# CSTR-Edinburgh/magphase

Hardware: AMD Instinct MI355X
Metric: frames/sec analysis+synthesis @48kHz FFT=4096 (higher is better)
Workload: dtype f32

## Files before the change

### include/magphase_hip.h

```cpp
#ifndef MAGPHASE_HIP_H
#define MAGPHASE_HIP_H

#include <stddef.h>
#include <stdint.h>

#ifdef __cplusplus
extern "C" {
#endif

#define MPX_ABI_VERSION 2

#define MPX_OK 0
#define MPX_ERR_ARG (-1)
#define MPX_ERR_HIP (-2)
#define MPX_ERR_HOST (-3)

int mpx_version(void);
const char* mpx_last_error(void);

size_t mpx_tables_bytes(int fft_len);
int mpx_tables_init(void* stream, int fft_len, void* tables);

int mpx_analysis_frames(void* stream, int fft_len, const void* tables, const float* sig,
                        const int64_t* frame_pos, const int32_t* frame_left, const int32_t* frame_right,
                        int64_t n_frames, float* out_mag, float* out_real, float* out_imag, int64_t ld);

size_t mpx_tables_f64_bytes(int fft_len);
int mpx_tables_f64_init(void* stream, int fft_len, void* tables);
int mpx_analysis_frames_f64(void* stream, int fft_len, const void* tables_f64, const float* sig,
                            const int64_t* frame_pos, const int32_t* frame_left, const int32_t* frame_right,
                            int64_t n_frames, float* out_mag, float* out_real, float* out_imag, int64_t ld,
                            const float* rows_in_use);

int mpx_analysis_frames_f64w(void* stream, int fft_len, const void* tables_f64, const float* sig,
                             const int64_t* frame_pos, const int32_t* frame_left, const int32_t* frame_right,
                             int64_t n_frames, float* out_mag, float* out_real, float* out_imag, int64_t ld,
                             const float* rows_in_use, const double* win_tab, int32_t win_cap);

int mpx_analysis_compressed_fused(void* stream, int fft_len, const void* tables_f64, const float* sig,
                                  const int64_t* frame_pos, const int32_t* frame_left, const int32_t* frame_right,
                                  int64_t n_frames, const double* win_tab, int32_t win_cap, const float* wpack,
                                  const float* whalf, int32_t mag_dim, int32_t phase_dim, const float* voiced,
                                  int32_t mag_fbank, float* out_mag, float* out_real, float* out_imag);
int mpx_analysis_compressed_fused_cr(void* stream, int fft_len, const void* tables_f64, const float* sig,
                                     const int64_t* frame_pos, const int32_t* frame_left, const int32_t* frame_right,
                                     int64_t n_frames, const double* win_tab, int32_t win_cap, const float* wpack,
                                     const float* whalf, int32_t mag_dim, int32_t phase_dim, const float* rows_in_use,
                                     const int32_t* row0, const int32_t* row1, const float* row_t, int64_t n_const,
// ... 359 lines not shown
```

### magphase_amd/_lib.py

```python
import ctypes
import threading
import os

_HERE = os.path.dirname(os.path.abspath(__file__))
LIB_PATH = os.path.join(_HERE, "libmagphase_hip.so")

vp, i32, i64, sz, f64 = ctypes.c_void_p, ctypes.c_int32, ctypes.c_int64, ctypes.c_size_t, ctypes.c_double
u32 = ctypes.c_uint32

PROTOTYPES = {
    "mpx_version": (i32, []),
    "mpx_last_error": (ctypes.c_char_p, []),
    "mpx_tables_bytes": (sz, [i32]),
    "mpx_tables_init": (i32, [vp, i32, vp]),
    "mpx_feat_ld": (i64, [i32]),
    "mpx_analysis_frames": (i32, [vp, i32] + [vp] * 5 + [i64, vp, vp, vp, i64]),
    "mpx_tables_f64_bytes": (sz, [i32]),
    "mpx_tables_f64_init": (i32, [vp, i32, vp]),
    "mpx_analysis_frames_f64": (i32, [vp, i32] + [vp] * 5 + [i64, vp, vp, vp, i64, vp]),
    "mpx_analysis_frames_f64w": (i32, [vp, i32] + [vp] * 5 + [i64, vp, vp, vp, i64, vp, vp, i32]),
    "mpx_analysis_compressed_fused": (i32, [vp, i32] + [vp] * 5 + [i64, vp, i32, vp, vp, i32, i32, vp, i32, vp, vp,
                                       vp]),
    "mpx_analysis_compressed_fused_cr": (i32, [vp, i32] + [vp] * 5 + [i64, vp, i32, vp, vp, i32, i32] + [vp] * 4 +
                                          [i64] + [vp] * 4),
    "mpx_analysis_compressed_fused_cr_work_bytes": (i64, [i32, i64]),
    "mpx_analysis_compressed_fused_tiles": (i32, [i32, i32, ctypes.POINTER(i32), ctypes.POINTER(i32)]),
    "mpx_analysis_compressed_fused_waves": (i32, []),
    "mpx_analysis_compressed_fused_layout": (i32, []),
    "mpx_analysis_compressed_fused_blocks_per_cu": (i32, [i32, i32]),
    "mpx_synthesis_lossless_frames": (i32, [vp, i32] + [vp] * 4 + [i64, vp, i64]),
    "mpx_ola_gather": (i32, [vp, i32, vp, i32] + [vp] * 4 + [i64, vp]),
    "mpx_synth_ola_slots": (i32, []),
    "mpx_synth_ola_slot_weights": (i32, [vp, i32]),
    "mpx_ola_strip_floats": (i64, [i32]),
    "mpx_synthesis_lossless_ola": (i32, [vp, i32] + [vp] * 5 + [i32, vp, vp, i32, vp, vp, vp, i64]),
    "mpx_synthesis_lossless_ola_lerp": (i32, [vp, i32] + [vp] * 8 + [i32, vp, vp, i32, vp, vp, vp, i64]),
    "mpx_rows_lerp": (i32, [vp, i32, vp, vp, vp, i64, vp, vp, vp, i64, vp, vp, vp, i64]),
    "mpx_synthesis_lossless_backward": (i32, [vp, i32, vp, vp, i64, vp, vp, vp, i64, vp, vp, vp, i64] + [vp] * 6 + [i64]),
    "mpx_synthesis_compressed_backward": (i32, [vp, i32, vp, vp, i64, vp, vp, vp, i64, vp, vp, vp, i64] + [vp] * 12
# ... 57 lines not shown
    "mpx_mel_unwarp_backward": (i32, [vp, i32, vp, i64, vp, i64, vp, i32, i64, vp, vp, vp, i64, i32, vp, i32, i64, vp, vp]),
    "mpx_phase_grad_mask": (i32, [vp, i64, i32] + [vp] * 7),
    "mpx_min_phase": (i32, [vp, i32] + [vp] * 5 + [i64, vp, vp, vp, i64]),
    "mpx_true_envelope": (i32, [vp, i32, vp, vp, vp, i64, i64, i32, f64, i32, vp, i64, vp, vp, vp]),
    "mpx_frame_gain": (i32, [vp, i32] + [vp] * 5 + [i64, vp, i32]),
    "mpx_noise_gains": (i32, [vp] * 4 + [i32, i32, vp, vp]),
    "mpx_noise_power": (i32, [vp, i32] + [vp] * 5 + [i64, vp]),
    "mpx_noise_rms": (i32, [vp, i32, vp, vp, i32, vp, vp]),
    "mpx_post_filter": (i32, [vp, vp, i64, i32, vp, i32, i32, vp, vp]),
    "mpx_epoch_f0_track": (i32, [vp, vp, vp, i32, i32, vp, i64, vp, vp, vp, i64] + [i32] * 4 + [f64, vp, vp, vp]),
    "mpx_epoch_zff": (i32, [vp, vp, vp, i32, i64, vp, i32, vp, vp, vp, i32] + [vp] * 5),
    "mpx_pcm16": (i32, [vp, vp, i32, vp, i32, i64, f64, vp, vp]),
    "mpx_pcm16_to_f32": (i32, [vp, vp, i64, vp]),
    "mpx_hpf_block": (i32, []),
    "mpx_output_hpf": (i32, [vp] * 4 + [i32, i64] + [vp] * 7),
    "mpx_bw_probe": (i32, [vp, i32, vp, vp, i64]),
    "mpx_bw_probe_shapes": (i32, []),
    "mpx_rows_pack": (i32, [vp, vp, vp, i32, i32] + [vp, i32, i64, i64] * 3),
    "mpx_post_filter_merlin": (i32, [vp, vp, i64, i32] + [vp] * 4 + [i32, f64, vp, f64] + [vp] * 5),
}
SYMBOLS = tuple(PROTOTYPES)
RT_STORE_FLAGS = {"rows": 4, "lines": 0, "lines_nt": 8}
RT_INVERSE_FLAGS = {"direct": 0, "transform": 32}
del vp, i32, i64, sz, f64

_lib = None


class MagphaseHipError(RuntimeError):
    pass


_load_lock = threading.Lock()


def load():
    global _lib
    if _lib is not None:
        return _lib
    with _load_lock:
        return _load_locked()


def _load_locked():
    global _lib
    if _lib is not None:
# ... 20 lines not shown
```

### magphase_amd/autograd.py

```python
import torch
from torch.autograd.function import once_differentiable


class _LosslessSynthesis(torch.autograd.Function):

    @staticmethod
    def forward(ctx, plan, cat_fn, n_utts, *mats):
        feats = [tuple(mats[3 * u:3 * u + 3]) for u in range(n_utts)]
        cat = cat_fn(feats)
        pcm = plan.run(cat[0], cat[1], cat[2])
        ctx.plan = plan
        ctx.rows = [int(f[0].shape[0]) for f in feats]
        ctx.like = [(m.dtype, tuple(m.shape)) if torch.is_tensor(m) else None for m in mats]
        ctx.save_for_backward(*cat)
        return pcm

    @staticmethod
    @once_differentiable
    def backward(ctx, grad_out):
        mag, real, imag = ctx.saved_tensors
        n_head = 3
        need_in = ctx.needs_input_grad[n_head:]
        need = tuple(any(need_in[k::3]) for k in range(3))
        if grad_out.dtype != torch.float32 or not grad_out.is_contiguous():
# ... 1 lines not shown
        with torch.cuda.device(grad_out.device):
            g = ctx.plan.run_backward(grad_out, mag, real, imag, need=need)
        out, a = [], 0
        for u, n in enumerate(ctx.rows):
            for k in range(3):
                like = ctx.like[3 * u + k]
                if like is None or not need_in[3 * u + k]:
                    out.append(None)
                else:
                    out.append(g[k][a:a + n].to(like[0]).reshape(like[1]))
            a += n
        return (None,) * n_head + tuple(out)


def synthesize(plan, cat_fn, feats):
    mats = [x for f in feats for x in f[:3]]
    return _LosslessSynthesis.apply(plan, cat_fn, len(feats), *mats)


class _LosslessAnalysis(torch.autograd.Function):

    @staticmethod
    def forward(ctx, plan, *sigs):
        mag, real, imag = plan.run()
        ctx.plan = plan
        ctx.like = [(s.dtype, tuple(s.shape)) if torch.is_tensor(s) else None for s in sigs]
        ctx.set_materialize_grads(False)
        ctx.save_for_backward(mag, real, imag)
        return mag, real, imag

    @staticmethod
    @once_differentiable
    def backward(ctx, *grads):
        mag, real, imag = ctx.saved_tensors
        need_in = ctx.needs_input_grad[1:]
        grads = tuple(g if g is None or (g.dtype == torch.float32 and g.is_contiguous())
                      else g.to(torch.float32).contiguous() for g in grads)
        with torch.cuda.device(mag.device):
            gsig = ctx.plan.run_backward(mag, real, imag, grads)
        out, a = [], 0
        for like, need, n in zip(ctx.like, need_in, ctx.plan.n_smpls):
            out.append(gsig[a:a + n].to(like[0]).reshape(like[1]) if like is not None and need else None)
            a += n
        return (None,) + tuple(out)


def analyze(plan, sigs):
# ... 112 lines not shown
```

### magphase_amd/csrc/magphase_hip.hip

```cpp
#include "mpx_common.hpp"

namespace mpx {

#ifdef MPX_ANA_NT
#define MPX_ST(dst, val) __builtin_nontemporal_store((val), &(dst))
#else
#define MPX_ST(dst, val) ((dst) = (val))
#endif

#ifndef MPX_ANA_QUEUE
#define MPX_ANA_QUEUE 0
#endif
template <int P>
__global__ __launch_bounds__(kAnaThreads) void k_analysis(const float* __restrict__ sig,
                                                          const long long* __restrict__ fpos,
                                                          const int* __restrict__ fleft,
                                                          const int* __restrict__ fright, long long nframes,
                                                          const float* __restrict__ tw_g, float* __restrict__ omag,
                                                          float* __restrict__ oreal, float* __restrict__ oimag,
                                                          long long ld) {
    constexpr int M = 64 * P, N = 2 * M, LB = ilog2(P), kTile = 64 * P;
    extern __shared__ __attribute__((aligned(16))) float smem[];
    float* tw = smem;
    const int lane_id = threadIdx.x & 63;
    const int wave = threadIdx.x >> 6;
    float* xbuf = smem + tw_floats<P>() + wave * (P * kXStride);
    const unsigned xbuf_byte = 4u * (unsigned)(tw_floats<P>() + rfl(wave) * (P * kXStride));
    for (int i = threadIdx.x; i < tw_floats<P>(); i += kAnaThreads) tw[i] = tw_g[i];
    unsigned* queue = reinterpret_cast<unsigned*>(smem + tw_floats<P>() + kAnaWaves * (P * kXStride));
    if (threadIdx.x == 0) *queue = 0u;
    __syncthreads();

    float wl_s0, wl_c0;
    sincospif(-2.0f * (float)kappa<P>(lane_id) / (float)N, &wl_s0, &wl_c0);

#if MPX_ANA_QUEUE
// ... 56 lines not shown
            }
            wave_sync();
        }

        wave_fft_front<P, -1>(re, im, tw, xbuf, lane);

#if MPX_ANA_QUEUE
        const long long fn = queue_pull(queue, fb);
#else
        const long long fn = f + fstep;
#endif
        FrameGeom gn = g;
        if (fn < fe) {
            gn = frame_geom(sig, fpos[fn], fleft[fn], fright[fn], N);
            asm volatile("s_waitcnt lgkmcnt(0)" ::: "memory");
            stage_samples_async(gn, 0, kTile, xbuf_byte, lane);
        }

        fft_inreg<P, -1>(re, im);

        float* row_m = omag + f * ld;
        float* row_r = oreal + f * ld;
        float* row_i = oimag + f * ld;
        float* mlo = row_m + kap;
        float* rlo = row_r + kap;
        float* ilo = row_i + kap;
        const int hoff = lane0 ? M - 64 : M - kap;
        float* mhi = row_m + hoff;
        float* rhi = row_r + hoff;
        float* ihi = row_i + hoff;
        float zpr[P / 2], zpi[P / 2];
#pragma unroll
        for (int q = 0; q < P / 2; ++q) {
            const int i = brev(q, LB);
            zpr[q] = __shfl(re[P - 1 - i], src_lane);
            zpi[q] = __shfl(im[P - 1 - i], src_lane);
        }
        float hm = 0.0f, hr = 0.0f, hi_ = 0.0f;
#pragma unroll
        for (int q = 0; q < P / 2; ++q) {
            const int i = brev(q, LB);
            const int i0 = brev((P - q) % P, LB);
            const float pr = lane0 ? re[i0] : zpr[q];
            const float pi = lane0 ? im[i0] : zpi[q];
            const float er = 0.5f * (re[i] + pr), ei = 0.5f * (im[i] - pi);
            const float orr = 0.5f * (im[i] + pi), oi = -0.5f * (re[i] - pr);
            const float cq = cos2p<P>(q), sq = -sin2p<P>(q);
            const float wr = wl_c * cq - wl_s * sq, wi = wl_c * sq + wl_s * cq;
            const float tr = wr * orr - wi * oi, ti = wr * oi + wi * orr;
            {
                const float xr = er + tr, xi = ei + ti;
                const float s2 = xr * xr + xi * xi;
                const float r = __builtin_amdgcn_rsqf(fmaxf(s2, 1.0e-37f));
#ifdef MPX_PROBE_NOSTORE
                asm volatile("" ::"v"(s2 * r), "v"(xr * r), "v"(xi * r));
#else
                MPX_ST(mlo[64 * q], s2 * r);
                MPX_ST(rlo[64 * q], xr * r);
                MPX_ST(ilo[64 * q], xi * r);
#endif
            }
            {
                const float xr = er - tr, xi = ti - ei;
                const float s2 = xr * xr + xi * xi;
                const float r = __builtin_amdgcn_rsqf(fmaxf(s2, 1.0e-37f));
                const float cm = s2 * r, cr = xr * r, ci = xi * r;
#ifdef MPX_PROBE_NOSTORE
                asm volatile("" ::"v"(cm), "v"(cr), "v"(ci));
#else
                if (q == 0) {
                    if (lane0) {
                        MPX_ST(row_m[M], cm);
                        MPX_ST(row_r[M], cr);
                        MPX_ST(row_i[M], ci);
                    }
                } else {
                    MPX_ST(mhi[-64 * (q - 1)], lane0 ? cm : hm);
                    MPX_ST(rhi[-64 * (q - 1)], lane0 ? cr : hr);
                    MPX_ST(ihi[-64 * (q - 1)], lane0 ? ci : hi_);
                }
#endif
                hm = cm;
                hr = cr;
                hi_ = ci;
            }
        }
        {
            const float xr = re[1], xi = -im[1];
            const float s2 = xr * xr + xi * xi;
            const float r = __builtin_amdgcn_rsqf(fmaxf(s2, 1.0e-37f));
#ifdef MPX_PROBE_NOSTORE
            asm volatile("" ::"v"(s2 * r), "v"(xr * r), "v"(xi * r), "v"(hm), "v"(hr), "v"(hi_));
#else
            MPX_ST(mhi[-64 * (P / 2 - 1)], lane0 ? s2 * r : hm);
            MPX_ST(rhi[-64 * (P / 2 - 1)], lane0 ? xr * r : hr);
            MPX_ST(ihi[-64 * (P / 2 - 1)], lane0 ? xi * r : hi_);
#endif
        }
        g = gn;
        if (fn >= fe) break;
#ifdef MPX_PROBE_NOSTORE
        staged_wait<0>();
#else
        staged_wait<3 * P + 3>();
#endif
        f = fn;
    }
}

template <int P>
__global__ __launch_bounds__(kThreads) void k_synth_lossless(const float* __restrict__ mag,
                                                             const float* __restrict__ real,
                                                             const float* __restrict__ imag, long long nframes,
                                                             const float* __restrict__ tw_g,
                                                             float* __restrict__ frames, long long ld) {
    constexpr int M = 64 * P, N = 2 * M, H = M + 1, LB = ilog2(P);
    extern __shared__ __attribute__((aligned(16))) float smem[];
    float* tw = smem;
    const int lane_id = threadIdx.x & 63;
    const int wave = threadIdx.x >> 6;
    float* xbuf = smem + tw_floats<P>() + wave * (P * kXStride);
    for (int i = threadIdx.x; i < tw_floats<P>(); i += kThreads) tw[i] = tw_g[i];
    __syncthreads();

    float wl_s0, wl_c0;
    sincospif(2.0f * (float)lane_id / (float)N, &wl_s0, &wl_c0);

// ... 557 lines not shown
        return fail(MPX_ERR_ARG, "mpx_analysis_frames: null pointer%s");
    const dim3 grid(grid_for(n_frames, kAnaWaves)), block(kAnaThreads);
    hipStream_t s = (hipStream_t)stream;
    if (P == 32) {
        if (int rc = set_lds(k_analysis<32>, lds_bytes_ana<32>())) return rc;
        hipLaunchKernelGGL(k_analysis<32>, grid, block, lds_bytes_ana<32>(), s, sig, (const long long*)frame_pos,
                           frame_left, frame_right, (long long)n_frames, (const float*)tables, out_mag, out_real,
                           out_imag, (long long)ld);
    } else if (P == 16) {
        if (int rc = set_lds(k_analysis<16>, lds_bytes_ana<16>())) return rc;
        hipLaunchKernelGGL(k_analysis<16>, grid, block, lds_bytes_ana<16>(), s, sig, (const long long*)frame_pos,
                           frame_left, frame_right, (long long)n_frames, (const float*)tables, out_mag, out_real,
                           out_imag, (long long)ld);
    } else {
        if (int rc = set_lds(k_analysis<8>, lds_bytes_ana<8>())) return rc;
        hipLaunchKernelGGL(k_analysis<8>, grid, block, lds_bytes_ana<8>(), s, sig, (const long long*)frame_pos,
                           frame_left, frame_right, (long long)n_frames, (const float*)tables, out_mag, out_real,
                           out_imag, (long long)ld);
    }
    MPX_HIP_CHECK(hipGetLastError());
    return MPX_OK;
}

int mpx_synthesis_lossless_frames(void* stream, int fft_len, const void* tables, const float* mag, const float* real,
                                  const float* imag, int64_t n_frames, float* frames_out, int64_t ld) {
    const int P = p_of(fft_len);
    if (!P) return fail(MPX_ERR_ARG, "mpx_synthesis_lossless_frames: fft_len must be 1024, 2048 or 4096%s");
    if (n_frames < 0) return fail(MPX_ERR_ARG, "mpx_synthesis_lossless_frames: negative n_frames%s");
    if (ld < fft_len / 2 + 1) return fail(MPX_ERR_ARG, "mpx_synthesis_lossless_frames: ld < fft_len/2 + 1%s");
    if (n_frames == 0) return MPX_OK;
    if (!tables || !mag || !real || !imag || !frames_out)
        return fail(MPX_ERR_ARG, "mpx_synthesis_lossless_frames: null pointer%s");
    const dim3 grid(grid_for(n_frames)), block(kThreads);
    hipStream_t s = (hipStream_t)stream;
    if (P == 32) {
        if (int rc = set_lds(k_synth_lossless<32>, lds_bytes<32>())) return rc;
        hipLaunchKernelGGL(k_synth_lossless<32>, grid, block, lds_bytes<32>(), s, mag, real, imag,
                           (long long)n_frames, (const float*)tables, frames_out, (long long)ld);
    } else if (P == 16) {
        if (int rc = set_lds(k_synth_lossless<16>, lds_bytes<16>())) return rc;
        hipLaunchKernelGGL(k_synth_lossless<16>, grid, block, lds_bytes<16>(), s, mag, real, imag,
                           (long long)n_frames, (const float*)tables, frames_out, (long long)ld);
    } else {
        if (int rc = set_lds(k_synth_lossless<8>, lds_bytes<8>())) return rc;
        hipLaunchKernelGGL(k_synth_lossless<8>, grid, block, lds_bytes<8>(), s, mag, real, imag,
                           (long long)n_frames, (const float*)tables, frames_out, (long long)ld);
// ... 218 lines not shown
```

### magphase_amd/csrc/wave_fft.hpp

```cpp
#pragma once
#include <hip/hip_runtime.h>

namespace mpx {

constexpr int kXStride = 68;

template <int P>
__host__ __device__ constexpr int tw_stride() { return 2 * P + 4; }
template <int P>
__host__ __device__ constexpr int tw_floats() { return 64 * tw_stride<P>(); }

__host__ __device__ constexpr int ilog2(int v) { return v <= 1 ? 0 : 1 + ilog2(v >> 1); }

__host__ __device__ constexpr int brev(int i, int bits) {
    int r = 0;
    for (int b = 0; b < bits; ++b) r |= ((i >> b) & 1) << (bits - 1 - b);
    return r;
}

__device__ __forceinline__ constexpr float c32(int k) {
    constexpr float t[16] = {1.000000000e+00f, 9.807852507e-01f, 9.238795042e-01f, 8.314695954e-01f,
                             7.071067691e-01f, 5.555702448e-01f, 3.826834261e-01f, 1.950903237e-01f,
                             0.0f,             -1.950903237e-01f, -3.826834261e-01f, -5.555702448e-01f,
                             -7.071067691e-01f, -8.314695954e-01f, -9.238795042e-01f, -9.807852507e-01f};
// ... 285 lines not shown
        if (upper) {
#pragma unroll
            for (int lp = 0; lp < P; ++lp) {
                const float xr = re[lp] * fc - im[lp] * fs;
                const float xi = re[lp] * fs + im[lp] * fc;
                re[lp] = xr;
                im[lp] = xi;
            }
        }
    }
    if (PARTNER == 2 * P) {
        if (rot) {
#pragma unroll
            for (int lp = 0; lp < P; ++lp) {
                const float xr = re[lp], xi = im[lp];
                re[lp] = (SIGN < 0) ? xi : -xi;
                im[lp] = (SIGN < 0) ? -xr : xr;
            }
        }
    }
}

template <int P>
__device__ __forceinline__ int kappa(int lane) {
    if (P == 32) return lane;
    if (P == 16) return (lane & 15) | (((lane >> 5) & 1) << 4) | (((lane >> 4) & 1) << 5);
    return (lane & 7) | (((lane >> 5) & 1) << 3) | (lane & 16) | (((lane >> 3) & 1) << 5);
}

template <int P, int SIGN>
__device__ __forceinline__ void wave_fft_front(float (&re)[P], float (&im)[P], const float* tw, float* xbuf, int lane) {
    fft_inreg<P, SIGN>(re, im);
    const float4* trow = reinterpret_cast<const float4*>(tw + lane * tw_stride<P>());
#pragma unroll
    for (int q = 0; q < P / 2; ++q) {
        const float4 w = trow[q];
#pragma unroll
        for (int e = 0; e < 2; ++e) {
            const int i = 2 * q + e;
            const float wc = e ? w.z : w.x;
            const float ws = (SIGN < 0) ? -(e ? w.w : w.y) : (e ? w.w : w.y);
            const float xr = re[i] * wc - im[i] * ws;
            const float xi = re[i] * ws + im[i] * wc;
            re[i] = xr;
            im[i] = xi;
        }
    }
// ... 216 lines not shown
```

### magphase_amd/engine.py

```python
import ctypes
import os

import numpy as np

from . import _lib, hostmath as hm, hostplan


def _torch():
    import torch

    return torch


class HostTicket:

    def __init__(self, ring, slot, event, keep):
        self._ring, self._slot, self._event, self._keep = ring, slot, event, keep

    def wait(self):
        if self._event is not None:
            self._event.synchronize()
            self._event = self._keep = None

    def release(self):
# ... 928 lines not shown
    def tables_f64(self, fft_len):
        key = ("f64", fft_len)
        if key not in self._tables:
            torch = _torch()
            nbytes = self.lib.mpx_tables_f64_bytes(int(fft_len))
            if nbytes == 0:
                raise ValueError("fft_len %r not supported by the HIP path (1024, 2048 or 4096)" % (fft_len,))
            t = torch.empty(nbytes // 8, dtype=torch.float64, device=self.device)
            self.launch("mpx_tables_f64_init", int(fft_len), t)
            self._tables[key] = t
        return self._tables[key]

    def hann_table(self):
        t = getattr(self, "_hann_table", None)
        if t is None:
            t = self._hann_table = self.to_device(hm.hann_half_table(), np.float64)
        return t

    def hann_window_args(self):
        if os.environ.get("MAGPHASE_F64_WINDOW", "table") == "analytic":
            return None, 0
        return self.hann_table(), hm.HANN_TABLE_CAP

    def analysis_frames(self, fft_len, sig, pos, left, right, out=None, precise=False, rows_in_use=None):
        nfr = int(pos.numel())
        H = fft_len // 2 + 1
        if out is None:
            out = tuple(self.empty_feats(nfr, H) for _ in range(3))
        ld = self.feat_ld(*out)
        if precise:
            self.launch("mpx_analysis_frames_f64w", int(fft_len), self.tables_f64(fft_len), sig, pos, left, right, nfr,
                        out[0], out[1], out[2], ld, rows_in_use, *self.hann_window_args())
        else:
            self.launch("mpx_analysis_frames", int(fft_len), self.tables(fft_len), sig, pos, left, right, nfr,
                        out[0], out[1], out[2], ld)
        return out

    def synthesis_lossless_frames(self, fft_len, mag, real, imag, out=None):
        nfr = int(mag.shape[0])
        if out is None:
            out = self.empty((nfr, fft_len))
        self.launch("mpx_synthesis_lossless_frames", int(fft_len), self.tables(fft_len), mag, real, imag, nfr, out,
                    self.feat_ld(mag, real, imag))
        return out

    def ola_gather(self, fft_len, frames, utt_frame_off, pm_rel, out_start, out_off, max_out_len, total_out, out=None):
        if out is None:
            out = self.empty((int(total_out),))
        self.launch("mpx_ola_gather", int(fft_len), frames, int(out_start.numel()), utt_frame_off, pm_rel, out_start,
                    out_off, int(max_out_len), out)
        return out

    def synth_ola_slots(self):
        torch = _torch()
        with torch.cuda.device(self.device):
            n = int(self.lib.mpx_synth_ola_slots())
        cus = os.environ.get("MAGPHASE_SYN_CUS")
        return n if not cus else max(6, min(n, 6 * int(cus)))
# ... 359 lines not shown
```

### magphase_amd/plans.py

```python
import ctypes
import os

import numpy as np

from . import _lib, hostmath as hm, hostplan


def _torch():
    import torch

    return torch


def _is_tensor(x):
    return type(x).__module__.startswith("torch") and _torch().is_tensor(x)


def _rows_or_array(engine, x, name):
    if not _is_tensor(x):
        return np.atleast_2d(np.asarray(x))
    hm.check_feature_tensor(x, name)
    if x.device.type == "cpu":
        x = x.detach()
        return (x.float() if x.element_size() == 2 else x).numpy()
# ... 112 lines not shown
    return (d.pop("row0"), d.pop("row1"), d.pop("rowt")), d


def _check_prepared(prepared, engine, utts):
    if prepared.n_utts != len(utts) or prepared.engine is not engine:
        prepared.release()
        raise ValueError("prepared: not the host side of this batch on this engine")


def _wait_ready(plan):
    ev = getattr(plan, "_ready", None)
    if ev is not None:
        _torch().cuda.current_stream(plan.engine.device).wait_event(ev)


def _widen_pcm16(engine, raw, total):
    sig = engine.empty((max(total, 1),))
    engine.launch("mpx_pcm16_to_f32", raw, total, sig)
    return sig[:total]


class LosslessAnalysisPlan:

    def __init__(self, engine, utts, fft_len=None, prepared=None, keep_frame_tabs=False):
        self.engine = engine
        self._keep_tabs = bool(keep_frame_tabs)
        utts, on_dev = _signal_inputs(engine, utts)
        if on_dev:
            if prepared is not None:
                prepared.release()
                raise ValueError("prepared= was built from host arrays: it cannot be combined with tensor inputs")
            self._from_device(engine, utts, fft_len)
            return
        if prepared is None and hasattr(engine, "prepare_analysis") and os.environ.get("MAGPHASE_NATIVE_PREPARE", "1") != "0":
            prepared = engine.prepare_analysis(utts, fft_len, wait=False)
        if prepared is not None:
            self._from_prepared(prepared, utts)
            return
        pos, left, right = [], [], []
        self.v_shift, self.v_f0, self.fs, self.n_frames, self.n_smpls, self.v_pm = [], [], [], [], [], []
        total = int(sum(np.shape(u[0])[0] for u in utts))
        staged = hasattr(engine, "host_staging")
        all_i16 = staged and len(utts) > 0 and all(np.asarray(u[0]).dtype == np.int16 for u in utts)
        if all_i16:
            buf = engine.host_staging((total + 1) // 2 + 2).view(np.int16)
        else:
            buf = engine.host_staging(total) if staged else np.empty(total, dtype=np.float32)
# ... 148 lines not shown
        self.long_frame_lens = [[] for _ in range(p.n_utts)]
        if p.long:
            utt_of = np.searchsorted(fo, [i for i, _n in p.long], side="right") - 1
            for (i, n), u in zip(p.long, utt_of.tolist()):
                self.long_frame_lens[u].append(n)
        F, total = p.total_frames, p.total_smpls
        o_pos, o_left, o_right, o_voi = p.offs
        if self._keep_tabs:
            d = p.slot["desc_np"]
            self._host_tabs = tuple(d[o:o + w * F].view(t).copy()
                                    for o, w, t in ((o_pos, 8, np.int64), (o_left, 4, np.int32), (o_right, 4, np.int32)))
        slot, p.slot = p.slot, None
        sd, dd, ev = e._slot_upload(slot, p.stage_bytes, p.desc_bytes)
        self._ready = ev
        if p.all_i16:
            self.sig = _widen_pcm16(e, sd, total)
        else:
            self.sig = sd[:4 * total].view(torch.float32)
        self.pos = dd[o_pos:o_pos + 8 * F].view(torch.int64)
        self.left = dd[o_left:o_left + 4 * F].view(torch.int32)
        self.right = dd[o_right:o_right + 4 * F].view(torch.int32)
        self.voi_dev = dd[o_voi:o_voi + 4 * F].view(torch.float32)

    def run(self, out=None, precise=False, rows_in_use=None):
        _wait_ready(self)
        return self.engine.analysis_frames(self.fft_len, self.sig, self.pos, self.left, self.right, out=out,
                                           precise=precise, rows_in_use=rows_in_use if precise else None)


class LosslessSynthesisPlan:

    def __init__(self, engine, f0_list, fs_list, fft_len, frames_per_run=None, comp_slots=False, gcuts=None, n_slots=None,
                 extents=None):
        n_slots_arg = n_slots
        self.engine = engine
        self.fft_len = fft_len
        pm_rel, starts, lens, nfr = [], [], [], []
        self.v_pm = []
        try:
            r = hostplan.plan_lossless_synthesis(f0_list, fs_list, fft_len)
            fo = r["frame_off"]
            for u in range(len(f0_list)):
                a, b = int(fo[u]), int(fo[u + 1])
                self.v_pm.append(r["v_pm"][a:b]), pm_rel.append(r["pm_rel"][a:b])
                starts.append(int(r["out_start"][u])), lens.append(int(r["out_len"][u])), nfr.append(b - a)
        except hostplan.PlanFallback:
            for v_f0, fs in zip(f0_list, fs_list):
                v_pm = np.cumsum(hm.f0_to_shift(np.asarray(v_f0, dtype=np.float64), fs)).astype(int)
                rel, start, out_len = hm.ola_plan(v_pm, fft_len)
                self.v_pm.append(v_pm)
# ... 133 lines not shown
                cuts, _t = hm.deal_cuts(terms, coef)
            except ValueError:
                return None
        self.deal = "cost"
        return cuts

    def run(self, feats=None, strips=None, out=None):
        e, a, s = self.engine, self.analysis, self.seams
        if feats is None:
            feats = tuple(e.empty_feats(self.total_frames, self.fft_len // 2 + 1) for _ in range(3))
        if out is None:
            out = e.empty((self.total_out,))
        if self.total_frames == 0:
            return feats, out
        _run_ola(e, lambda strips, out: e.roundtrip_lossless_ola(self.fft_len, a, s, feats, strips, out,
                                                                 full_support=self.full_support, stores=self.stores,
                                                                 inverse=self.inverse),
                 self.fft_len, s, strips, out, self.total_out)
        return feats, out


class LosslessConstRateAnalysisPlan:

    def __init__(self, engine, utts, fft_len=None, const_rate_ms=5.0, prepared=None):
        self.engine = e = engine
        self.const_rate_ms = hm.check_const_rate_ms(const_rate_ms)
        self.lossless = pl = LosslessAnalysisPlan(engine, utts, fft_len=fft_len, prepared=prepared)
        self.fft_len, self.fs, self.long_frame_lens = pl.fft_len, pl.fs, pl.long_frame_lens
        U = len(utts)
        self.row0_host, self.row1_host, self.rowt_host, self.v_f0, self.out_off = hm.var_to_const_rate_batch(
            [pl.v_shift[u] for u in range(U)], [pl.v_f0[u] for u in range(U)], pl.frame_off[:U], pl.fs,
            self.const_rate_ms)
        self.total_out_frames = int(self.out_off[-1])
        self.rows, _ = _upload_rows(e, (self.row0_host, self.row1_host, self.rowt_host))

    def run(self, out=None):
        e = self.engine
        H = self.fft_len // 2 + 1
        if out is None:
            out = tuple(e.empty_feats(self.total_out_frames, H) for _ in range(3))
        if self.total_out_frames == 0:
            return out
        var = self.lossless.run()
        e.rows_lerp(var, self.rows, self.total_out_frames, out=out)
        del var
        return out


class LosslessConstRateSynthesisPlan:

    def __init__(self, engine, f0_list, fs_list, fft_len, const_rate_ms=5.0, frames_per_run=None, host=None):
        self.engine = e = engine
        self.fft_len = int(fft_len)
        self.const_rate_ms = hm.check_const_rate_ms(const_rate_ms)
        r = host if host is not None else hostplan.plan_const_rate_synthesis(f0_list, fs_list, self.const_rate_ms)
        self.live, self.n_rows = r["live"], r["n_rows"]
        self.v_shift, self.v_locs, self.v_voi, self.v_f0 = r["v_shift"], r["v_locs"], r["v_voi"], r["v_f0"]
        self.row0_host, self.row1_host, self.rowt_host = r["row0"], r["row1"], r["rowt"]
        self.total_rows = int(sum(self.n_rows))
        self.inner = None
        out_len = [0] * len(self.n_rows)
        if self.live:
            self.inner = LosslessSynthesisPlan(e, self.v_f0, [fs_list[u] for u in self.live], self.fft_len,
                                               frames_per_run=frames_per_run)
            for k, u in enumerate(self.live):
                out_len[u] = self.inner.out_len[k]
# ... 715 lines not shown

        if self.fused:
            out = outputs()
            e.launch("mpx_analysis_compressed_fused", N, e.tables_f64(N), pl.sig, pl.pos, pl.left, pl.right,
                     int(pl.total_frames), *e.hann_window_args(), self.wpack, self.whalf, self.mag_dim, self.phase_dim,
                     self.voi, fbank, out[0], out[1], out[2])
            mark("k_analysis_warp_fused")
            return out
        n_var = int(pl.total_frames)
        if self.fused_cr:
            out = outputs()
            self._phase_rows_tmp()
            if self._cr_work is None:
                nbytes = int(e.lib.mpx_analysis_compressed_fused_cr_work_bytes(N, n_var))
                self._cr_work = e.empty(((nbytes + 3) // 4,))
            e.launch("mpx_analysis_compressed_fused_cr", N, e.tables_f64(N), pl.sig, pl.pos, pl.left, pl.right, n_var,
                     *e.hann_window_args(), self.wpack, self.whalf, self.mag_dim, self.phase_dim, self.rows_in_use,
                     self.row0, self.row1, self.rowt, int(Fo), out[0], *self._phase_tmp, self._cr_work)
            mark("k_analysis_warp_fused_cr")
            e.launch("mpx_warp_phase_rows", int(Fo), self.phase_dim, *self._phase_tmp, self.row0, self.row1, self.rowt,
                     self.voi, out[1], out[2])
            mark("k_warp_phase_rows")
            return out
        mag, real, imag = pl.run(out=feats, precise=precise, rows_in_use=self.rows_in_use if self.phase_on_rows else None)
        mark("k_analysis_f64" if precise else "k_analysis")
        out = outputs()
        warp = (Fo, H, mag, real, imag, self.row0, self.row1, self.rowt, self.w_mag, self.mag_dim, self.w_ph, self.phase_dim,
                self.voi, out[0], out[1], out[2], e.feat_ld(mag, real, imag))
        if self.phase_on_rows:
            e.launch("mpx_mel_warp_rows", *warp, fbank, n_var, self.rows_in_use, *self._phase_rows_tmp())
        else:
            e.launch(self._warp_name, *warp)
        mark("k_mel_warp_mfma")
        return out

    def run_backward(self, outs, grads, mark=None):
        if self._warp_name == "mpx_mel_warp_fbank":
            raise NotImplementedError("the filter-bank magnitudes (b_mag_fbank_mel) have no backward pass")
        torch = _torch()
        e, pl, N = self.engine, self.lossless, int(self.fft_len)
        H = N // 2 + 1
        Fo, n_var, total = self.total_out_frames, int(pl.total_frames), int(pl.total_smpls)
        mark = mark or (lambda name: None)
        mark("start")
        shapes = ((Fo, self.mag_dim), (Fo, self.phase_dim), (Fo, self.phase_dim))
        for g, shp in zip(grads, shapes):
            if g is not None and (g.dtype != torch.float32 or tuple(g.shape) != shp or not g.is_contiguous()):
                raise ValueError("run_backward: gradients must be contiguous float32 of the outputs' shapes")
        g_m, g_r, g_i = grads
        if Fo == 0 or n_var == 0 or total == 0 or all(g is None for g in grads):
            return torch.zeros((total,), dtype=torch.float32, device=e.device)
        precise = os.environ.get("MAGPHASE_COMP_ANALYSIS", "f64") != "f32"
        rows = pl.run(precise=precise, rows_in_use=None)
        mark("rows")
        h_r, h_i = e.phase_grad_mask(outs[1], outs[2], self.voi, g_r, g_i)
        tabs = live = None
        if self.b_const_rate:
            if getattr(self, "_adj", None) is None:
                r0, r1, rt = self._rows_host
                self._adj = e.to_device(hm.lerp_adjoint_table(r0, r1, rt, n_var).reshape(-1), np.int32)
            tabs = (self.row0, self.row1, self.rowt)
            _none, h_r, h_i = e.rows_lerp_adjoint((None, h_r, h_i), self._adj, self.rowt, n_var)
            live = self.rows_in_use
        else:
            live = self.voi
        mark("k_phase_grad_mask")
        have_ph = h_r is not None or h_i is not None
        g_rows = e.mel_warp_backward(H, mag=(g_m, self.w_mag, rows[0], tabs) if g_m is not None else None,
                                     phase=(h_r, h_i, self.w_ph, rows[1], rows[2], live) if have_ph else None)
        mark("k_mel_warp_bwd")
        if self.b_const_rate and g_rows[0] is not None:
            g_rows = (e.rows_lerp_adjoint((g_rows[0], None, None), self._adj, self.rowt, n_var)[0],) + tuple(g_rows[1:])
            mark("k_rows_lerp_adjoint")
        gsig = pl.run_backward(rows[0], rows[1], rows[2], g_rows)
        mark("k_analysis_lossless_bwd")
        return gsig
# ... 112 lines not shown
```

Measured before the change: 184.5 million.

## Add cache-line-aligned and nontemporal store modes to the FFT-4096 analysis kernel

```diff
diff --git a/include/magphase_hip.h b/include/magphase_hip.h
--- a/include/magphase_hip.h
+++ b/include/magphase_hip.h
@@ -24,6 +24,12 @@
 int mpx_analysis_frames(void* stream, int fft_len, const void* tables, const float* sig,
                         const int64_t* frame_pos, const int32_t* frame_left, const int32_t* frame_right,
                         int64_t n_frames, float* out_mag, float* out_real, float* out_imag, int64_t ld);
+
+#define MPX_ANA_STORE_LINES 1
+#define MPX_ANA_STORE_NT 2
+int mpx_analysis_frames_flags(void* stream, int fft_len, const void* tables, const float* sig,
+                              const int64_t* frame_pos, const int32_t* frame_left, const int32_t* frame_right,
+                              int64_t n_frames, float* out_mag, float* out_real, float* out_imag, int64_t ld, int flags);
 
 size_t mpx_tables_f64_bytes(int fft_len);
 int mpx_tables_f64_init(void* stream, int fft_len, void* tables);
diff --git a/magphase_amd/_lib.py b/magphase_amd/_lib.py
--- a/magphase_amd/_lib.py
+++ b/magphase_amd/_lib.py
@@ -15,6 +15,7 @@
     "mpx_tables_init": (i32, [vp, i32, vp]),
     "mpx_feat_ld": (i64, [i32]),
     "mpx_analysis_frames": (i32, [vp, i32] + [vp] * 5 + [i64, vp, vp, vp, i64]),
+    "mpx_analysis_frames_flags": (i32, [vp, i32] + [vp] * 5 + [i64, vp, vp, vp, i64, i32]),
     "mpx_tables_f64_bytes": (sz, [i32]),
     "mpx_tables_f64_init": (i32, [vp, i32, vp]),
     "mpx_analysis_frames_f64": (i32, [vp, i32] + [vp] * 5 + [i64, vp, vp, vp, i64, vp]),
@@ -118,6 +119,7 @@
 SYMBOLS = tuple(PROTOTYPES)
 RT_STORE_FLAGS = {"rows": 4, "lines": 0, "lines_nt": 8}
 RT_INVERSE_FLAGS = {"direct": 0, "transform": 32}
+ANA_STORE_FLAGS = {"rows": 0, "lines": 1, "lines_nt": 3}
 del vp, i32, i64, sz, f64
 
 _lib = None
diff --git a/magphase_amd/autograd.py b/magphase_amd/autograd.py
--- a/magphase_amd/autograd.py
+++ b/magphase_amd/autograd.py
@@ -47,7 +47,7 @@
 
     @staticmethod
     def forward(ctx, plan, *sigs):
-        mag, real, imag = plan.run()
+        mag, real, imag = plan.run(read_back=True)
         ctx.plan = plan
         ctx.like = [(s.dtype, tuple(s.shape)) if torch.is_tensor(s) else None for s in sigs]
         ctx.set_materialize_grads(False)
diff --git a/magphase_amd/csrc/magphase_hip.hip b/magphase_amd/csrc/magphase_hip.hip
--- a/magphase_amd/csrc/magphase_hip.hip
+++ b/magphase_amd/csrc/magphase_hip.hip
@@ -2,16 +2,18 @@
 
 namespace mpx {
 
-#ifdef MPX_ANA_NT
-#define MPX_ST(dst, val) __builtin_nontemporal_store((val), &(dst))
-#else
-#define MPX_ST(dst, val) ((dst) = (val))
-#endif
+constexpr int kAnaStoreRows = 0, kAnaStoreLines = 1, kAnaStoreLinesNT = 2;
+template <int P>
+constexpr bool kappa_is_identity() {
+    for (int l = 0; l < 64; ++l)
+        if (kappa<P>(l) != l) return false;
+    return true;
+}
 
 #ifndef MPX_ANA_QUEUE
 #define MPX_ANA_QUEUE 0
 #endif
-template <int P>
+template <int P, int ST = kAnaStoreRows>
 __global__ __launch_bounds__(kAnaThreads) void k_analysis(const float* __restrict__ sig,
                                                           const long long* __restrict__ fpos,
                                                           const int* __restrict__ fleft,
@@ -114,13 +116,40 @@
         float* row_m = omag + f * ld;
         float* row_r = oreal + f * ld;
         float* row_i = oimag + f * ld;
-        float* mlo = row_m + kap;
-        float* rlo = row_r + kap;
-        float* ilo = row_i + kap;
+        static_assert(ST == kAnaStoreRows || P == 32, "the line-aligned store forms exist for P = 32 only");
+        static_assert(ST == kAnaStoreRows || kappa_is_identity<P>(), "by line: lane l holds bins l + 64 q");
+        int s_m = 0, s_r = 0, s_i = 0;
+        if constexpr (ST != kAnaStoreRows) {
+            s_m = __builtin_amdgcn_readfirstlane(row_store_phase(row_m));
+            s_r = __builtin_amdgcn_readfirstlane(row_store_phase(row_r));
+            s_i = __builtin_amdgcn_readfirstlane(row_store_phase(row_i));
+        }
+        const bool pv_m = row_asc_prev(kap, s_m), pv_r = row_asc_prev(kap, s_r), pv_i = row_asc_prev(kap, s_i);
+        const bool cu_m = row_mir_cur(kap, s_m), cu_r = row_mir_cur(kap, s_r), cu_i = row_mir_cur(kap, s_i);
+        unsigned long long k_pv_m = 0, k_pv_r = 0, k_pv_i = 0, k_cu_m = 0, k_cu_r = 0, k_cu_i = 0;
+        if constexpr (ST != kAnaStoreRows) {
+            k_pv_m = __builtin_amdgcn_ballot_w64(pv_m), k_cu_m = __builtin_amdgcn_ballot_w64(cu_m);
+            k_pv_r = __builtin_amdgcn_ballot_w64(pv_r), k_cu_r = __builtin_amdgcn_ballot_w64(cu_r);
+            k_pv_i = __builtin_amdgcn_ballot_w64(pv_i), k_cu_i = __builtin_amdgcn_ballot_w64(cu_i);
+        }
+        auto st_line = [](float* dst, float v) {
+            if constexpr (ST == kAnaStoreLinesNT) __builtin_nontemporal_store(v, dst);
+            else *dst = v;
+        };
+        auto st_mask = [](float* dst, float v, unsigned long long mask) {
+            unsigned long long saved;
+            asm volatile("s_and_saveexec_b64 %0, %3\n\tglobal_store_dword %1, %2, off\n\ts_mov_b64 exec, %0"
+                         : "=&s"(saved)
+                         : "v"(dst), "v"(v), "s"(mask)
+                         : "memory", "scc");
+        };
+        float* mlo = row_m + (ST != kAnaStoreRows ? 0 : kap);
+        float* rlo = row_r + (ST != kAnaStoreRows ? 0 : kap);
+        float* ilo = row_i + (ST != kAnaStoreRows ? 0 : kap);
         const int hoff = lane0 ? M - 64 : M - kap;
-        float* mhi = row_m + hoff;
-        float* rhi = row_r + hoff;
-        float* ihi = row_i + hoff;
+        float* mhi = row_m + (ST != kAnaStoreRows ? 0 : hoff);
+        float* rhi = row_r + (ST != kAnaStoreRows ? 0 : hoff);
+        float* ihi = row_i + (ST != kAnaStoreRows ? 0 : hoff);
         float zpr[P / 2], zpi[P / 2];
 #pragma unroll
         for (int q = 0; q < P / 2; ++q) {
@@ -129,6 +158,7 @@
             zpi[q] = __shfl(im[P - 1 - i], src_lane);
         }
         float hm = 0.0f, hr = 0.0f, hi_ = 0.0f;
+        float pm = 0.0f, pr_ = 0.0f, pi_ = 0.0f;
 #pragma unroll
         for (int q = 0; q < P / 2; ++q) {
             const int i = brev(q, LB);
@@ -147,9 +177,25 @@
 #ifdef MPX_PROBE_NOSTORE
                 asm volatile("" ::"v"(s2 * r), "v"(xr * r), "v"(xi * r));
 #else
-                MPX_ST(mlo[64 * q], s2 * r);
-                MPX_ST(rlo[64 * q], xr * r);
-                MPX_ST(ilo[64 * q], xi * r);
+                if constexpr (ST == kAnaStoreRows) {
+                    mlo[64 * q] = s2 * r;
+                    rlo[64 * q] = xr * r;
+                    ilo[64 * q] = xi * r;
+                } else {
+                    const float om = s2 * r, orl = xr * r, oim = xi * r;
+                    if (q == 0) {
+                        st_mask(mlo + row_asc_base(kap, false) + row_asc_off(0), om, ~k_pv_m);
+                        st_mask(rlo + row_asc_base(kap, false) + row_asc_off(0), orl, ~k_pv_r);
+                        st_mask(ilo + row_asc_base(kap, false) + row_asc_off(0), oim, ~k_pv_i);
+                    } else {
+                        st_line(mlo + row_asc_base(kap, pv_m) + row_asc_off(q), pv_m ? pm : om);
+                        st_line(rlo + row_asc_base(kap, pv_r) + row_asc_off(q), pv_r ? pr_ : orl);
+                        st_line(ilo + row_asc_base(kap, pv_i) + row_asc_off(q), pv_i ? pi_ : oim);
+                    }
+                    pm = om;
+                    pr_ = orl;
+                    pi_ = oim;
+                }
 #endif
             }
             {
@@ -160,16 +206,28 @@
 #ifdef MPX_PROBE_NOSTORE
                 asm volatile("" ::"v"(cm), "v"(cr), "v"(ci));
 #else
-                if (q == 0) {
-                    if (lane0) {
-                        MPX_ST(row_m[M], cm);
-                        MPX_ST(row_r[M], cr);
-                        MPX_ST(row_i[M], ci);
+                if constexpr (ST == kAnaStoreRows) {
+                    if (q == 0) {
+                        if (lane0) {
+                            row_m[M] = cm;
+                            row_r[M] = cr;
+                            row_i[M] = ci;
+                        }
+                    } else {
+                        mhi[-64 * (q - 1)] = lane0 ? cm : hm;
+                        rhi[-64 * (q - 1)] = lane0 ? cr : hr;
+                        ihi[-64 * (q - 1)] = lane0 ? ci : hi_;
+                    }
+                } else if (q == 0) {
+                    if (cu_m || cu_r || cu_i) {
+                        st_mask(mhi + row_mir_base(kap, true, M) + row_mir_off(0), cm, k_cu_m);
+                        st_mask(rhi + row_mir_base(kap, true, M) + row_mir_off(0), cr, k_cu_r);
+                        st_mask(ihi + row_mir_base(kap, true, M) + row_mir_off(0), ci, k_cu_i);
                     }
                 } else {
-                    MPX_ST(mhi[-64 * (q - 1)], lane0 ? cm : hm);
-                    MPX_ST(rhi[-64 * (q - 1)], lane0 ? cr : hr);
-                    MPX_ST(ihi[-64 * (q - 1)], lane0 ? ci : hi_);
+                    st_line(mhi + row_mir_base(kap, cu_m, M) + row_mir_off(q), cu_m ? cm : hm);
+                    st_line(rhi + row_mir_base(kap, cu_r, M) + row_mir_off(q), cu_r ? cr : hr);
+                    st_line(ihi + row_mir_base(kap, cu_i, M) + row_mir_off(q), cu_i ? ci : hi_);
                 }
 #endif
                 hm = cm;
@@ -184,9 +242,20 @@
 #ifdef MPX_PROBE_NOSTORE
             asm volatile("" ::"v"(s2 * r), "v"(xr * r), "v"(xi * r), "v"(hm), "v"(hr), "v"(hi_));
 #else
-            MPX_ST(mhi[-64 * (P / 2 - 1)], lane0 ? s2 * r : hm);
-            MPX_ST(rhi[-64 * (P / 2 - 1)], lane0 ? xr * r : hr);
-            MPX_ST(ihi[-64 * (P / 2 - 1)], lane0 ? xi * r : hi_);
+            if constexpr (ST == kAnaStoreRows) {
+                mhi[-64 * (P / 2 - 1)] = lane0 ? s2 * r : hm;
+                rhi[-64 * (P / 2 - 1)] = lane0 ? xr * r : hr;
+                ihi[-64 * (P / 2 - 1)] = lane0 ? xi * r : hi_;
+            } else {
+                st_mask(mlo + row_asc_base(kap, true) + row_asc_off(P / 2), pm, k_pv_m);
+                st_mask(rlo + row_asc_base(kap, true) + row_asc_off(P / 2), pr_, k_pv_r);
+                st_mask(ilo + row_asc_base(kap, true) + row_asc_off(P / 2), pi_, k_pv_i);
+                static_assert(row_mir_tail_live(0, true) && !row_mir_tail_live(1, true) && row_mir_tail_live(1, false),
+                              "the mirror tail's lanes: lane 0 and those that do not store this step's mirror");
+                st_mask(mhi + row_mir_base(kap, cu_m, M) + row_mir_off(P / 2), lane0 ? s2 * r : hm, ~k_cu_m | 1ull);
+                st_mask(rhi + row_mir_base(kap, cu_r, M) + row_mir_off(P / 2), lane0 ? xr * r : hr, ~k_cu_r | 1ull);
+                st_mask(ihi + row_mir_base(kap, cu_i, M) + row_mir_off(P / 2), lane0 ? xi * r : hi_, ~k_cu_i | 1ull);
+            }
 #endif
         }
         g = gn;
@@ -194,7 +263,7 @@
 #ifdef MPX_PROBE_NOSTORE
         staged_wait<0>();
 #else
-        staged_wait<3 * P + 3>();
+        staged_wait<ST == kAnaStoreRows ? 3 * P + 3 : 3 * row_store_count(P)>();
 #endif
         f = fn;
     }
@@ -798,6 +867,40 @@
     return MPX_OK;
 }
 
+int mpx_analysis_frames_flags(void* stream, int fft_len, const void* tables, const float* sig, const int64_t* frame_pos,
+                              const int32_t* frame_left, const int32_t* frame_right, int64_t n_frames, float* out_mag,
+                              float* out_real, float* out_imag, int64_t ld, int flags) {
+    const int P = p_of(fft_len);
+    if (!P) return fail(MPX_ERR_ARG, "mpx_analysis_frames_flags: fft_len must be 1024, 2048 or 4096%s");
+    if (flags & ~(MPX_ANA_STORE_LINES | MPX_ANA_STORE_NT))
+        return fail(MPX_ERR_ARG, "mpx_analysis_frames_flags: unknown flag bits%s");
+    if ((flags & MPX_ANA_STORE_NT) && !(flags & MPX_ANA_STORE_LINES))
+        return fail(MPX_ERR_ARG, "mpx_analysis_frames_flags: MPX_ANA_STORE_NT needs MPX_ANA_STORE_LINES%s");
+    if (n_frames < 0) return fail(MPX_ERR_ARG, "mpx_analysis_frames_flags: negative n_frames%s");
+    if (ld < fft_len / 2 + 1) return fail(MPX_ERR_ARG, "mpx_analysis_frames_flags: ld < fft_len/2 + 1%s");
+    if (n_frames == 0) return MPX_OK;
+    if (!tables || !sig || !frame_pos || !frame_left || !frame_right || !out_mag || !out_real || !out_imag)
+        return fail(MPX_ERR_ARG, "mpx_analysis_frames_flags: null pointer%s");
+    if (P != 32 || !(flags & MPX_ANA_STORE_LINES))
+        return mpx_analysis_frames(stream, fft_len, tables, sig, frame_pos, frame_left, frame_right, n_frames, out_mag,
+                                   out_real, out_imag, ld);
+    const dim3 grid(grid_for(n_frames, kAnaWaves)), block(kAnaThreads);
+    hipStream_t s = (hipStream_t)stream;
+    if (flags & MPX_ANA_STORE_NT) {
+        if (int rc = set_lds(k_analysis<32, kAnaStoreLinesNT>, lds_bytes_ana<32>())) return rc;
+        hipLaunchKernelGGL((k_analysis<32, kAnaStoreLinesNT>), grid, block, lds_bytes_ana<32>(), s, sig,
+                           (const long long*)frame_pos, frame_left, frame_right, (long long)n_frames, (const float*)tables,
+                           out_mag, out_real, out_imag, (long long)ld);
+    } else {
+        if (int rc = set_lds(k_analysis<32, kAnaStoreLines>, lds_bytes_ana<32>())) return rc;
+        hipLaunchKernelGGL((k_analysis<32, kAnaStoreLines>), grid, block, lds_bytes_ana<32>(), s, sig,
+                           (const long long*)frame_pos, frame_left, frame_right, (long long)n_frames, (const float*)tables,
+                           out_mag, out_real, out_imag, (long long)ld);
+    }
+    MPX_HIP_CHECK(hipGetLastError());
+    return MPX_OK;
+}
+
 int mpx_synthesis_lossless_frames(void* stream, int fft_len, const void* tables, const float* mag, const float* real,
                                   const float* imag, int64_t n_frames, float* frames_out, int64_t ld) {
     const int P = p_of(fft_len);
diff --git a/magphase_amd/csrc/wave_fft.hpp b/magphase_amd/csrc/wave_fft.hpp
--- a/magphase_amd/csrc/wave_fft.hpp
+++ b/magphase_amd/csrc/wave_fft.hpp
@@ -331,7 +331,7 @@
 }
 
 template <int P>
-__device__ __forceinline__ int kappa(int lane) {
+__host__ __device__ __forceinline__ constexpr int kappa(int lane) {
     if (P == 32) return lane;
     if (P == 16) return (lane & 15) | (((lane >> 5) & 1) << 4) | (((lane >> 4) & 1) << 5);
     return (lane & 7) | (((lane >> 5) & 1) << 3) | (lane & 16) | (((lane >> 3) & 1) << 5);
diff --git a/magphase_amd/engine.py b/magphase_amd/engine.py
--- a/magphase_amd/engine.py
+++ b/magphase_amd/engine.py
@@ -974,7 +974,9 @@
             return None, 0
         return self.hann_table(), hm.HANN_TABLE_CAP
 
-    def analysis_frames(self, fft_len, sig, pos, left, right, out=None, precise=False, rows_in_use=None):
+    def analysis_frames(self, fft_len, sig, pos, left, right, out=None, precise=False, rows_in_use=None, stores="rows"):
+        if stores not in _lib.ANA_STORE_FLAGS:
+            raise ValueError("stores must be rows, lines or lines_nt, not %r" % (stores,))
         nfr = int(pos.numel())
         H = fft_len // 2 + 1
         if out is None:
@@ -984,8 +986,8 @@
             self.launch("mpx_analysis_frames_f64w", int(fft_len), self.tables_f64(fft_len), sig, pos, left, right, nfr,
                         out[0], out[1], out[2], ld, rows_in_use, *self.hann_window_args())
         else:
-            self.launch("mpx_analysis_frames", int(fft_len), self.tables(fft_len), sig, pos, left, right, nfr,
-                        out[0], out[1], out[2], ld)
+            self.launch("mpx_analysis_frames_flags", int(fft_len), self.tables(fft_len), sig, pos, left, right, nfr,
+                        out[0], out[1], out[2], ld, _lib.ANA_STORE_FLAGS[stores])
         return out
 
     def synthesis_lossless_frames(self, fft_len, mag, real, imag, out=None):
diff --git a/magphase_amd/plans.py b/magphase_amd/plans.py
--- a/magphase_amd/plans.py
+++ b/magphase_amd/plans.py
@@ -158,7 +158,24 @@
 
 class LosslessAnalysisPlan:
 
+    DEFAULT_STORES = "lines_nt"
+    READ_BACK_STORES = "lines"
+
+    @staticmethod
+    def _stores(default):
+        s = os.environ.get("MAGPHASE_ANA_STORES", "") or default
+        if s not in _lib.ANA_STORE_FLAGS:
+            raise ValueError("MAGPHASE_ANA_STORES must be rows, lines or lines_nt, not %r" % (s,))
+        return s
+
     def __init__(self, engine, utts, fft_len=None, prepared=None, keep_frame_tabs=False):
+        try:
+            self.stores = self._stores(self.DEFAULT_STORES)
+            self.read_back_stores = self._stores(self.READ_BACK_STORES)
+        except ValueError:
+            if prepared is not None:
+                prepared.release()
+            raise
         self.engine = engine
         self._keep_tabs = bool(keep_frame_tabs)
         utts, on_dev = _signal_inputs(engine, utts)
@@ -353,10 +370,11 @@
         self.right = dd[o_right:o_right + 4 * F].view(torch.int32)
         self.voi_dev = dd[o_voi:o_voi + 4 * F].view(torch.float32)
 
-    def run(self, out=None, precise=False, rows_in_use=None):
+    def run(self, out=None, precise=False, rows_in_use=None, read_back=False):
         _wait_ready(self)
         return self.engine.analysis_frames(self.fft_len, self.sig, self.pos, self.left, self.right, out=out,
-                                           precise=precise, rows_in_use=rows_in_use if precise else None)
+                                           precise=precise, rows_in_use=rows_in_use if precise else None,
+                                           stores=self.read_back_stores if read_back else self.stores)
 
 
 class LosslessSynthesisPlan:
@@ -536,6 +554,8 @@
 
 class LosslessConstRateAnalysisPlan:
 
+    DEFAULT_STORES = LosslessAnalysisPlan.READ_BACK_STORES
+
     def __init__(self, engine, utts, fft_len=None, const_rate_ms=5.0, prepared=None):
         self.engine = e = engine
         self.const_rate_ms = hm.check_const_rate_ms(const_rate_ms)
@@ -555,7 +575,7 @@
             out = tuple(e.empty_feats(self.total_out_frames, H) for _ in range(3))
         if self.total_out_frames == 0:
             return out
-        var = self.lossless.run()
+        var = self.lossless.run(read_back=True)
         e.rows_lerp(var, self.rows, self.total_out_frames, out=out)
         del var
         return out
@@ -1317,7 +1337,8 @@
                      self.voi, out[1], out[2])
             mark("k_warp_phase_rows")
             return out
-        mag, real, imag = pl.run(out=feats, precise=precise, rows_in_use=self.rows_in_use if self.phase_on_rows else None)
+        mag, real, imag = pl.run(out=feats, precise=precise, rows_in_use=self.rows_in_use if self.phase_on_rows else None,
+                                 read_back=True)
         mark("k_analysis_f64" if precise else "k_analysis")
         out = outputs()
         warp = (Fo, H, mag, real, imag, self.row0, self.row1, self.rowt, self.w_mag, self.mag_dim, self.w_ph, self.phase_dim,
@@ -1346,7 +1367,7 @@
         if Fo == 0 or n_var == 0 or total == 0 or all(g is None for g in grads):
             return torch.zeros((total,), dtype=torch.float32, device=e.device)
         precise = os.environ.get("MAGPHASE_COMP_ANALYSIS", "f64") != "f32"
-        rows = pl.run(precise=precise, rows_in_use=None)
+        rows = pl.run(precise=precise, rows_in_use=None, read_back=True)
         mark("rows")
         h_r, h_i = e.phase_grad_mask(outs[1], outs[2], self.voi, g_r, g_i)
         tabs = live = None
```

Result: no change. 183.7 million (-0.4%).
